# yoshihikosuzuki/ClassPro

Hardware: AMD Instinct MI355X
Metric: Mbases/s classified (k=40, 40x HiFi) at 1/2/4/8 MI355X vs CPU -T16 (higher is better)
Workload: dtype u16/f64

## Files before the change

classpro_amd/csrc/capi.hip:

```cpp
#include <hip/hip_runtime.h>
#include <stdio.h>
#include <stdlib.h>
#include <string.h>
#include <string>
#include <mutex>
#include <vector>
#include <chrono>
#include <thread>
#include <type_traits>
#include <time.h>
#include "cp_host_setup.h"
#include "kernels.hip"

static thread_local std::string g_err;
static int set_err(int code, const std::string &msg) { g_err = msg; return code; }

#define HIPCHK(call)                                                                       \
  do { hipError_t e_ = (call);                                                             \
       if (e_ != hipSuccess)                                                               \
         return set_err(CP_EHIP,std::string(#call)+": "+hipGetErrorString(e_));            \
     } while (0)
static int launch_status() { HIPCHK(hipGetLastError()); return CP_OK; }

extern "C" const char *cp_last_error(void) { return g_err.c_str(); }
// ... 964 lines not shown
  unsigned long long z[4] = { 0, 0, 0, 0 };
  HIPCHK(hipMemcpyToSymbol(HIP_SYMBOL(g_bounds),z,sizeof(z)));
  return CP_OK;
}
#endif

#if defined(CP_SEED_DEBUG) || defined(CP_SEED_DEBUG_TAKES)
extern "C" int cp_debug_seed_set(int read)
{ HIPCHK(hipMemcpyToSymbol(HIP_SYMBOL(g_seed_dbg_read),&read,sizeof(int))); return CP_OK; }
extern "C" int cp_debug_seed_get(int *out4, int *recs)
{ HIPCHK(hipDeviceSynchronize());
  HIPCHK(hipMemcpyFromSymbol(out4,HIP_SYMBOL(g_seed_dbg_n),16));
  HIPCHK(hipMemcpyFromSymbol(recs,HIP_SYMBOL(g_seed_dbg),8192*16));
  return CP_OK;
}
#endif
#if defined(CP_SEED_PROF) || defined(CP_PROF_WALK)
static int prof_read(unsigned long long *out, const void *sym, size_t n, bool reset = true)
{ static const unsigned long long z[12] = {0};
  HIPCHK(hipMemcpyFromSymbol(out,sym,n*sizeof(unsigned long long)));
  if (reset) HIPCHK(hipMemcpyToSymbol(sym,z,n*sizeof(unsigned long long)));
  return CP_OK;
}
#endif
#ifdef CP_SEED_PROF
extern "C" int cp_debug_seed_prof(unsigned long long *out8)
{ HIPCHK(hipDeviceSynchronize()); return prof_read(out8,HIP_SYMBOL(g_seed_prof),8); }
#endif
extern "C" int cp_debug_task_counts(cp_workspace *ws, int32_t *out, int64_t nreads)
{ if (!ws || !out || nreads < 0 || nreads > ws->nreads || ws->b.fwc.cap < (size_t)nreads*16)
    return set_err(CP_EINVAL,"cp_debug_task_counts: bad arguments");
  HIPCHK(hipDeviceSynchronize());
  if (nreads > 0) HIPCHK(hipMemcpy(out,ws->b.fwc.p,(size_t)nreads*4*sizeof(int32_t),hipMemcpyDeviceToHost));
  return CP_OK;
}
extern "C" int cp_debug_flag_bytes(cp_workspace *ws, int64_t *out2)
{ if (!ws || !out2) return set_err(CP_EINVAL,"cp_debug_flag_bytes: bad arguments");
  HIPCHK(hipDeviceSynchronize());
  const dbuf *arr[2] = { &ws->b.wall, &ws->b.wall_s };
  for (int a = 0; a < 2; a++)
    { std::vector<uint8_t> h(arr[a]->cap);
      if (arr[a]->cap) HIPCHK(hipMemcpy(h.data(),arr[a]->p,arr[a]->cap,hipMemcpyDeviceToHost));
      int64_t n = 0;
      for (uint8_t v : h) n += v != 0;
      out2[a] = n;
    }
  return CP_OK;
}
#ifdef CP_PROF_WALK
extern "C" int cp_debug_live_prof(unsigned long long *out8)
{ HIPCHK(hipDeviceSynchronize()); return prof_read(out8,HIP_SYMBOL(g_live_prof),8); }
extern "C" int cp_debug_emit_prof(unsigned long long *out8)
{ HIPCHK(hipDeviceSynchronize()); return prof_read(out8,HIP_SYMBOL(g_emit_prof),8); }
extern "C" int cp_debug_unrel_prof(unsigned long long *out8)
{ HIPCHK(hipDeviceSynchronize()); return prof_read(out8,HIP_SYMBOL(g_unrel_prof),8); }
extern "C" int cp_debug_rel_prof(unsigned long long *out12)
{ HIPCHK(hipDeviceSynchronize()); return prof_read(out12,HIP_SYMBOL(g_rel_prof),12); }
extern "C" int cp_debug_phase_prof(unsigned long long *out36)
{ HIPCHK(hipDeviceSynchronize());
  CHK(prof_read(out36,HIP_SYMBOL(g_phase_max),12));
  CHK(prof_read(out36+12,HIP_SYMBOL(g_phase_sum),12));
  return prof_read(out36+24,HIP_SYMBOL(g_phase_arg),12,false);
}
#endif

#include "kmer_table.hip"

#include "kmer_counts.hip"

#include "kmer_sort.hip"

#include "kmer_lookup.hip"

#include "kmer_hits.hip"

#include "kmer_runs.hip"

#include "kmer_setops.hip"

#include "kmer_cmphist.hip"

#include "kmer_hetpairs.hip"

#include "label_tools.hip"
```

classpro_amd/csrc/kernels.hip:

```cpp
#include <hip/hip_runtime.h>
#include <stdint.h>
#include <type_traits>
#include "cp_wall.h"
#include "cp_class.h"
#include "cp_seed.h"

#ifdef CP_BOUNDS
__device__ unsigned long long g_bounds[4];
#endif
#define WAVE 64
#define REL_MAXM 1024
#define UNREL_MAXN 1024
#ifndef REL_SMALL_MAXM
#define REL_SMALL_MAXM 112
#endif
#ifndef UNREL_SMALL_MAXN
#define UNREL_SMALL_MAXN 256
#endif
#define GRP_MAX_PLEN 65535

__device__ __forceinline__ void wave_sync() { __syncthreads(); }
__device__ __forceinline__ void wave_sync_lds()
{ __builtin_amdgcn_fence(__ATOMIC_RELEASE,"wavefront"); __builtin_amdgcn_wave_barrier(); __builtin_amdgcn_fence(__ATOMIC_ACQUIRE,"wavefront"); }

// ... 630 lines not shown
            }
          if (mv != ~0ull) break;
        }
      if (nx > 0 && !done && !flush_x(right ? 0x7fffffff : -1)) return;
      if (!done && (right ? plen < jend : jend == 0))
        { const double pe = pe_i * pe_i;
          if (pe >= CP_PE_THRES_FINAL)
            { if (*midx >= R->ecap) { R->overflow = 1; return; }
              ev.wave_grow(*midx);
              if (lane == 0)
                { cp_eintvl x; x.b = right ? i : 0; x.e = right ? plen : i; x.pe = pe;
                  ev.put(*midx,x);
                  F.fo[q] |= CP_W_PAIRED_M;
                }
              (*midx)++;
              if (*midx >= plen) { R->overflow = 8; return; }
            }
        }
      wave_sync();
    }
}

#define CP_PCLS(e,a)   (((uint32_t)(e) << 3) | ((uint32_t)(a) & 7u))
#define CP_PCLS_END(x) ((int)((x) >> 3))
#define CP_PCLS_CLS(x) (((x) & 7u) == 7u ? -1 : (int)((x) & 7u))

struct cp_rrec { int32_t b, e; uint16_t ccb, cce; int32_t idx; double pe; };
static_assert(sizeof(cp_rrec) == 24,"compact reliable-interval record");
struct cp_ivA { int32_t b, e; uint16_t cb, ce, ccb, cce; };
struct cp_ivB { double pe, peo_b, peo_e; };
struct cp_ivC { uint8_t is_rel; int8_t asgn; };
static_assert(sizeof(cp_ivA) == 16 && sizeof(cp_ivB) == 24 && sizeof(cp_ivC) == 2,"interval records as arrays");
struct cp_soa { cp_ivA *a; cp_ivB *b; cp_ivC *c; };
__device__ __forceinline__ void cp_soa_put(const cp_soa &S, int64_t at, const cp_intvl &I)
{ cp_ivA a; a.b = I.b; a.e = I.e; a.cb = I.cb; a.ce = I.ce; a.ccb = I.ccb; a.cce = I.cce;
  cp_ivB b; b.pe = I.pe; b.peo_b = I.peo_b; b.peo_e = I.peo_e;
  cp_ivC c; c.is_rel = I.is_rel; c.asgn = I.asgn;
  S.a[at] = a; S.b[at] = b; S.c[at] = c;
}
__device__ __forceinline__ cp_intvl cp_soa_get(const cp_soa &S, int64_t at)
{ const cp_ivA a = S.a[at]; const cp_ivB b = S.b[at]; const cp_ivC c = S.c[at];
  cp_intvl I;
  memset(&I,0,sizeof(I));
  I.b = a.b; I.e = a.e; I.cb = a.cb; I.ce = a.ce; I.ccb = a.ccb; I.cce = a.cce;
  I.is_rel = c.is_rel; I.asgn = c.asgn; I.pe = b.pe; I.peo_b = b.peo_b; I.peo_e = b.peo_e;
  return I;
}

#ifdef CP_PROF_WALK
__device__ unsigned long long g_phase_max[12], g_phase_sum[12], g_phase_arg[12];
__device__ unsigned long long g_live_prof[8];
__device__ unsigned long long g_unrel_prof[8];
__device__ unsigned long long g_emit_prof[8];
#ifdef CP_PROF_INNER
#define EM_LT0() unsigned long long em_t = wall_clock64()
#define EM_LT(k) do { unsigned long long t_ = wall_clock64(); if (lane == 0) atomicAdd(&g_emit_prof[k],t_-em_t); em_t = wall_clock64(); } while (0)
#endif
#define PH_STAMP(k) do { if (lane == 0) { unsigned long long t_ = wall_clock64(); unsigned long long d_ = t_-ph_t; ph_t = t_; \
      atomicAdd(&g_phase_sum[k],d_); unsigned long long o_ = atomicMax(&g_phase_max[k],d_); if (d_ > o_) g_phase_arg[k] = ((unsigned long long)r << 32) | (unsigned)n_c; } } while (0)
#elif defined(CP_STOP_AT)
#define PH_STAMP(k) do { if ((k) == CP_STOP_AT) { PH_STOP_EXTRA; return; } } while (0)
#else
#define PH_STAMP(k) ((void)0)
#endif
#ifndef EM_LT0
#define EM_LT0() ((void)0)
#define EM_LT(k) ((void)0)
#endif
#define PH_STOP_EXTRA

struct task_res { double own_pe, lc_v, hc_pe; int lc_j, hc;  };

#define FW_SEQ_WIN    32
#define FW_SEQ_STRIDE 36
struct cp_seq_lwin
  { CP_SEQ_T g; CP_LDS_PTR(const char) w; int lo, len;
    __device__ __forceinline__ char operator[](int p) const
    { const unsigned d = (unsigned)(p-lo); return d < (unsigned)len ? w[d] : g[p]; }
  };
__device__ __forceinline__ int cp_seq_dirword(const cp_seq_lwin &sq, int rlen, int pos, int dir, uint64_t *D)
{ (void)rlen;
  const int d = (dir > 0 ? pos : pos-7)-sq.lo;
  if (d < 0 || d+8 > sq.len) return 0;
  CP_LDS_PTR(const uint32_t) rw = (CP_LDS_PTR(const uint32_t))(sq.w+(d & ~3));
  const uint32_t x0 = rw[0], x1 = rw[1], x2 = rw[2];
  const uint32_t sh = (uint32_t)(d & 3)*8;
  const uint32_t lo = __builtin_amdgcn_alignbit(x1,x0,sh), hi = __builtin_amdgcn_alignbit(x2,x1,sh);
  const uint64_t x = (uint64_t)lo | ((uint64_t)hi << 32);
  *D = dir > 0 ? x : __builtin_bswap64(x);
  return 8;
}
struct __attribute__((packed, aligned(1))) cp_u8x16 { uint32_t v[4]; };
struct __attribute__((packed, aligned(1))) cp_u8x4 { uint32_t v; };
struct cp_seq_rwin
  { CP_SEQ_T g;
    uint64_t wl, wh;
    int lo, len;
    __device__ __forceinline__ char operator[](int p) const
    { const unsigned d = (unsigned)(p-lo);
      if (d < (unsigned)len)
        { const uint64_t x = (d < 8) ? wl : wh;
          return (char)(x >> ((d & 7)*8));
        }
      return g[p];
    }
  };
__device__ __forceinline__ int cp_seq_dirword(const cp_seq_rwin &sq, int rlen, int pos, int dir, uint64_t *D)
{ (void)rlen;
  const int d = (dir > 0 ? pos : pos-7)-sq.lo;
  if (sq.len != 16 || d < 0 || d > 8) return 0;
  const uint64_t x = d == 0 ? sq.wl : d == 8 ? sq.wh : (sq.wl >> (8*d)) | (sq.wh << (64-8*d));
  *D = dir > 0 ? x : __builtin_bswap64(x);
  return 8;
}
struct cp_seq_rsrc { CP_SEQ_T g; };
__device__ __forceinline__ cp_seq_rwin cp_seq_window(const cp_seq_rsrc &src, int pos, int rlen, int dir)
{ cp_seq_rwin sq;
  int lo = dir > 0 ? pos-7 : pos-11;
  if (lo > rlen-16) lo = rlen-16;
  if (lo < 0) lo = 0;
  sq.g = src.g; sq.lo = lo; sq.len = 0; sq.wl = sq.wh = 0;
  if (rlen-lo >= 16)
    { const cp_u8x16 x = *reinterpret_cast<const cp_u8x16 *>(CP_SPAN(src.g,lo,16));
      sq.wl = (uint64_t)x.v[0] | ((uint64_t)x.v[1] << 32);
// ... 51 lines not shown
  R.seq.g = CP_SEQ_VIEW(seq+seq_off[r],rlen); R.seq.w = (CP_LDS_PTR(const char))(s_win+lane*FW_SEQ_STRIDE); R.seq.lo = 0; R.seq.len = 0;
  R.wall = wall_all+po+r; R.wall_s = R.wall;
  R.eintvl = R.ointvl = nullptr; R.ecap = 0; R.eidx = R.oidx = 0; R.overflow = 0;
  cp_read_t<cp_perr_hybrid,cp_seq_rwin> R1;
  R1.P = P; R1.prof = R.prof; R1.lf = P->logfact; R1.plen = plen; R1.rlen = rlen;
  R1.wall = R.wall; R1.wall_s = R.wall; R1.eintvl = R1.ointvl = nullptr; R1.ecap = 0; R1.eidx = R1.oidx = 0; R1.overflow = 0;
  const int icap = (int)(ioff[r+1]-ioff[r]);
  int32_t *wl = wlist+ioff[r]*4;
  task_res *tres = tres_all+ioff[r];
  uint8_t *wall = R.wall;
  int32_t *cinfo = wl, *clist = wl+icap, *ccnt = wl+2*(int64_t)icap, *tlist = wl+3*(int64_t)icap;
  int n_c = 0;
#ifdef CP_PROF_WALK
  unsigned long long ph_t = wall_clock64();
#endif
  if (plen > 1)
    { const int64_t lo = po+1, hi = po+plen;
      const int64_t w_lo = lo >> 6, w_hi = (hi-1) >> 6;
      for (int64_t wb = w_lo; wb <= w_hi; wb += WAVE)
        { const int64_t w = wb+lane;
          const uint64_t bits = (w <= w_hi) ? bitmap_word(bm,w,lo,hi) : 0ull;
          int c = __popcll(bits), off = c;
          for (int o = 1; o < WAVE; o <<= 1)
            { int x = __shfl_up(off,o); if (lane >= o) off += x; }
          const int tot = __shfl(off,WAVE-1);
          off = n_c+off-c;
          for (uint64_t t = bits; t; t &= t-1)
            { const int k = __ffsll((long long)t)-1;
              if (off < icap) clist[off] = (int)((w << 6)+k-po);
              if (off < FW_LISTS) s_cl[off] = (int)((w << 6)+k-po);
              off++;
            }
          n_c += tot;
        }
    }
  if (n_c > icap) n_c = icap;
  const bool lists = n_c <= FW_LISTS;
  if (lists) wave_sync_lds(); else wave_sync();
  PH_STAMP(0);
  int n_t = 0, n_live0 = 0;
  for (int base = 0; base < n_c; base += WAVE)
    { int f0 = 0, f1 = 0;
      if (!lists) { if (base+lane < n_c) s_cl[lane] = clist[base+lane]; wave_sync_lds(); }
      if (base+lane < n_c)
        { const int i = s_cl[lists ? base+lane : lane];
          const bool drop = R.prof[i-1] > R.prof[i];
          cp_seq_rsrc rs; rs.g = R.seq.g;
          R1.seq = cp_seq_window(rs,drop ? i+P->K-2 : i,rlen,drop ? -1 : +1);
          cp_wall_pre pre;
          cp_wall_candidate_pre(&R1,i,&pre);
          f0 = cp_wall_candidate_filter(P,CP_SELF,pre);
          f1 = cp_wall_candidate_filter(P,CP_OTHERS,pre);
          cinfo[base+lane] = pre.maxt*32+pre.maxl+(f0 << 8)+(f1 << 12);
          ccnt[base+lane] = (int)R.prof[i-1] | ((int)R.prof[i] << 16);
          if (lists)
            { s_ci[base+lane] = (uint16_t)(pre.maxt*32+pre.maxl+(f0 << 8)+(f1 << 12));
              s_cc[base+lane] = (int)R.prof[i-1] | ((int)R.prof[i] << 16);
            }
        }
      const int l0 = (f0 & CP_CF_LIVE) ? 1 : 0, l1 = (f1 & CP_CF_LIVE) ? 1 : 0;
      int c = l0+l1, off = c;
      for (int o = 1; o < WAVE; o <<= 1)
        { int x = __shfl_up(off,o); if (lane >= o) off += x; }
      const int tot = __shfl(off,WAVE-1);
      off = n_t+off-c;
      if (l0) { if (off < icap) tlist[off] = (base+lane)*2;   if (lists) s_tl[off] = (uint16_t)((base+lane)*2);   off++; }
      if (l1) { if (off < icap) tlist[off] = (base+lane)*2+1; if (lists) s_tl[off] = (uint16_t)((base+lane)*2+1); }
      n_t += tot;
      n_live0 += __popcll(__ballot(l0));
    }
  int ovf = 0;
  if (n_t > icap) { ovf = 1; n_t = 0; n_c = 0; }
  if (lists) wave_sync_lds(); else wave_sync();
  PH_STAMP(7);
  for (int tb = 0; tb < n_t; tb += WAVE)
    { const int nb = (n_t-tb < WAVE) ? n_t-tb : WAVE;
      if (lane < nb)
        { if (!lists)
            { const int code = tlist[tb+lane], k = code >> 1;
              s_tl[lane] = (uint16_t)(lane*2+(code & 1)); s_cl[lane] = clist[k]; s_ci[lane] = (uint16_t)cinfo[k]; s_cc[lane] = ccnt[k];
            }
          const int code = s_tl[lists ? tb+lane : lane], k = code >> 1, e = code & 1;
          const int i = s_cl[k], tl = s_ci[k] & 255, cc = s_cc[k];
          cp_wall_pre pre;
          const int cim1 = cc & 0xffff, ci = (cc >> 16) & 0xffff;
          pre.cng = cim1 > ci ? cim1-ci : ci-cim1;
          if (cim1 > ci) { pre.wtype = CP_DROP; pre.cin = ci;   pre.cout = cim1; }
          else           { pre.wtype = CP_GAIN; pre.cin = cim1; pre.cout = ci;   }
          pre.maxt = tl >> 5; pre.maxl = tl & 31;
          pre.maxpe = P->pe[pre.maxt][pre.maxl];
          pre.lpe   = P->lpe[pre.maxt][pre.maxl];
          pre.l1mpe = P->l1mpe[pre.maxt][pre.maxl];
          cp_cand_pure c;
          cp_wall_candidate_live(&R,i,e,pre,&c,[&]() { fr_seq_win_load(R.seq,s_win+lane*FW_SEQ_STRIDE,cim1 > ci ? i+P->K-16 : i-24,rlen); });
          task_res q;
          q.own_pe = c.own_pe; q.lc_v = c.lc_v; q.hc_pe = c.hc_pe;
          q.lc_j = c.lc_j;
          q.hc = c.lc_kind | (c.hc_j >= 0 ? 4 : 0) | ((c.hc_j >= 0 ? c.hc_j-i : 0) << 16);
          tres[tb+lane] = q;
        }
    }
  PH_STAMP(6);
  if (lane == 0) { fwc[4*(int64_t)r] = n_c; fwc[4*(int64_t)r+1] = n_t; fwc[4*(int64_t)r+2] = n_live0; fwc[4*(int64_t)r+3] = ovf; }
}

#undef PH_STOP_EXTRA
#define PH_STOP_EXTRA
#ifndef FW2_WAVES_PER_EU
#define FW2_WAVES_PER_EU 5
#endif
__global__ void __launch_bounds__(WAVE) __attribute__((amdgpu_waves_per_eu(FW2_WAVES_PER_EU)))
k_find_wall(const cp_dev_params *__restrict__ P, const char *__restrict__ seq, const int64_t *__restrict__ seq_off,
            const uint16_t *__restrict__ prof, const int64_t *__restrict__ prof_off, int nreads,
            uint8_t *__restrict__ wall_all, uint8_t *__restrict__ walls_all,
            int32_t *__restrict__ hkeys, double *__restrict__ hvals, const int64_t *__restrict__ hoff,
            cp_eintvl *__restrict__ eintvl_all, cp_eintvl *__restrict__ ointvl_all, const int64_t *__restrict__ eoff,
            cp_intvl *__restrict__ intvl_all, const int64_t *__restrict__ ioff,
            int32_t *__restrict__ nintvl, int32_t *__restrict__ err, const int32_t *__restrict__ perm,
            int32_t *__restrict__ wlist, const task_res *__restrict__ tres_all, const int32_t *__restrict__ fwc,
            cp_intvl *__restrict__ rintvl_all, int32_t *__restrict__ relmap_all, int32_t *__restrict__ nrel, int do_rel,
            cp_rrec *__restrict__ rrec_all, cp_soa soa)
{ if ((int)blockIdx.x >= nreads) return;
  const int r = perm[blockIdx.x];
  const int lane = lane_id();
  const int64_t po = prof_off[r];
  const int plen = (int)(prof_off[r+1]-po);
  const int rlen = (int)(seq_off[r+1]-seq_off[r]);

#ifndef FW_XCAP
#define FW_XCAP 8
#endif
#ifndef FW_LCAP1
#define FW_LCAP1 64
#endif
  if (plen <= 0)
    { if (lane == 0) { nintvl[r] = 0; if (do_rel) nrel[r] = 0; }
      return;
    }
  constexpr int LCAP0 = 256, LCAP1 = FW_LCAP1;
  __shared__ int32_t s_mkey[LCAP0+LCAP1];
  __shared__ double  s_mval[LCAP0+LCAP1];
  __shared__ uint16_t s_x[FW_XCAP];
  __shared__ int s_nx;
  __shared__ cp_eintvl s_ev[FW_EVL];
  cp_read_t<cp_perr_hybrid,CP_SEQ_T,CP_PROF_T,const double *,fw_evl> R;
  R.P = P; R.prof = CP_PROF_VIEW(prof+po,plen); R.seq = CP_SEQ_VIEW(seq+seq_off[r],rlen); R.lf = P->logfact; R.plen = plen; R.rlen = rlen;
  R.wall = wall_all+po+r;
  R.wall_s = walls_all+po+r;
  { const int64_t ho = hoff[r], hc = (hoff[r+1]-ho) >> 1;
    R.perror.g.keys = hkeys+ho;
    R.perror.g.vals = hvals+ho*4;
    R.perror.g.mask = (uint32_t)hc-1;
    R.perror.lkeys = (CP_LDS_PTR(int32_t))s_mkey;
    R.perror.lvals = (CP_LDS_PTR(double))s_mval;
    R.perror.lcap0 = LCAP0; R.perror.lcap1 = LCAP1;
    R.perror.use_lds = 0;
  }
  if (lane == 0) s_nx = 0;
  for (int k = lane; k < LCAP0+LCAP1; k += WAVE)
    s_mkey[k] = -1;
  R.eintvl.g = eintvl_all+eoff[r];
  R.eintvl.l = (CP_LDS_PTR(cp_eintvl))s_ev;
  R.ointvl.g = ointvl_all+eoff[r];
  R.ecap = (int)(eoff[r+1]-eoff[r]);
  R.eidx = R.oidx = 0; R.overflow = 0;
  cp_intvl *intvl = intvl_all+ioff[r];
  const int icap = (int)(ioff[r+1]-ioff[r]);
  int32_t *wl = wlist+ioff[r]*4;
  const task_res *tres = tres_all+ioff[r];
  uint8_t *wall = R.wall;
  const uint8_t *wall_s = R.wall_s;
  __shared__ task_res s_res[WAVE];
  int32_t *clist = wl+icap, *ccnt = wl+2*(int64_t)icap, *tlist = wl+3*(int64_t)icap;
  const int n_c = fwc[4*(int64_t)r], n_t = fwc[4*(int64_t)r+1], n_live0 = fwc[4*(int64_t)r+2];
  if (fwc[4*(int64_t)r+3]) R.overflow = 1;
#ifdef CP_PROF_WALK
  unsigned long long ph_t = wall_clock64();
#endif
  R.perror.use_lds = ((2*n_live0 <= LCAP0-8) ? 1 : 0) | ((2*(n_t-n_live0) <= LCAP1-8) ? 2 : 0);
  R.eintvl.big = (n_live0 > FW_EVL || R.ecap < FW_EVL) ? 1 : 0;
  { const int hc = (int)R.perror.g.mask+1;
    for (int e = 0; e < 2; e++)
      if (!((R.perror.use_lds >> e) & 1))
        for (int k = lane; k < hc; k += WAVE) R.perror.g.keys[(size_t)e*hc+k] = -1;
  }
  wave_sync();
  int *sbuf = reinterpret_cast<int *>(s_res);
  constexpr int SBUF = (int)(sizeof(task_res)*WAVE/sizeof(int));
  constexpr int SCOMP = 64;
  constexpr int U16 = 2*(SBUF-2*SCOMP);
  uint16_t *s16 = reinterpret_cast<uint16_t *>(sbuf);
  fw_cflags F;
  F.pos = s16; F.fo = reinterpret_cast<uint8_t *>(s16+n_c); F.fs = F.fo+n_c; F.n = n_c;
  constexpr int NDEP = 128;
  static_assert(sizeof(task_res)*WAVE >= 4*256+NDEP*sizeof(unsigned long long),"flags of 255 candidates and the dependency masks fit the staging block");
  bool onchip = R.perror.use_lds == 3 && plen <= 65535 && n_c <= 255 && 3*n_c+2*SCOMP+1 <= U16 && !R.eintvl.big;
  const int32_t *cinfo = wl;
  auto flags_to_hbm = [&]()
    { for (int q = lane; q < n_c; q += WAVE)
        if ((cinfo[q] >> 12) & CP_CF_WALLNOW) wall[clist[q]] = CP_W_WALL_O;
      wave_sync();
    };
  if (R.perror.use_lds == 3)
    { unsigned long long *s_dep = reinterpret_cast<unsigned long long *>(s_res)+(sizeof(task_res)*WAVE/sizeof(unsigned long long)-NDEP);
      const uint64_t ltm = (1ull << lane)-1;
      const int ecap = R.ecap;
      const bool ebig = R.eintvl.big != 0;
      int eidx = 0, oidx = 0, ovf = 0;
      auto memo_cell = [&](int pos, int e, int w) -> int
        { const int key = pos*2+w, off = e ? LCAP0 : 0;
          const uint32_t m = (uint32_t)(e ? LCAP1 : LCAP0)-1;
          uint32_t h = ((uint32_t)key*0x9E3779B1u >> 9) & m;
          while (true)
            { const int32_t k = s_mkey[off+h];
              if (k == key) break;
              if (k < 0)
                { const int32_t o = atomicCAS(&s_mkey[off+h],-1,key);
                  if (o == -1) { s_mval[off+h] = -INFINITY; break; }
                  if (o == key) break;
                }
              h = (h+1) & m;
            }
          return off+(int)h;
        };
      for (;;)
        { if (onchip)
            { for (int q = lane; q < n_c; q += WAVE)
                { F.pos[q] = (uint16_t)clist[q]; F.fo[q] = ((cinfo[q] >> 12) & CP_CF_WALLNOW) ? CP_W_WALL_O : 0; F.fs[q] = 0; }
              wave_sync();
            }
          else flags_to_hbm();
          bool bail = false;
          for (int tb = 0; tb < n_t; tb += WAVE)
            { const int nb = (n_t-tb < WAVE) ? n_t-tb : WAVE;
              bool open = lane < nb;
              int pos = 1, kc = 0, e = 0, w = 0, lc_j = -1, lc_kind = CP_LC_NONE, hc_j = -1;
              double own_pe = 0., lc_v = 0., hc_pe = 0.;
              if (open)
                { const int code = tlist[tb+lane], k = code >> 1, cc = ccnt[k];
                  const task_res q = tres[tb+lane];
                  pos = clist[k]; kc = k; e = code & 1;
                  w = (cc & 0xffff) > ((cc >> 16) & 0xffff) ? CP_DROP : CP_GAIN;
                  own_pe = q.own_pe; lc_v = q.lc_v; hc_pe = q.hc_pe;
                  lc_j = q.lc_j; lc_kind = q.hc & 3;
                  hc_j = (q.hc & 4) ? pos+(q.hc >> 16) : -1;
                }
              const int p1 = (lc_kind == CP_LC_PAIR || lc_kind == CP_LC_BOUNDARY) ? lc_j : -1, p2 = hc_j;
              for (int q = lane; q < NDEP; q += WAVE) s_dep[q] = 0ull;
              wave_sync();
              const int s0 = (int)((uint32_t)(pos*2+e)*0x9E3779B1u >> 25), s1 = (int)((uint32_t)(p1*2+e)*0x9E3779B1u >> 25),
                        s2 = (int)((uint32_t)(p2*2+e)*0x9E3779B1u >> 25);
              if (open)
                { atomicOr(&s_dep[s0],1ull << lane);
                  if (p1 >= 0) atomicOr(&s_dep[s1],1ull << lane);
                  if (p2 >= 0) atomicOr(&s_dep[s2],1ull << lane);
                }
              wave_sync();
              uint64_t dep = 0;
              if (open)
                { dep = s_dep[s0];
                  if (p1 >= 0) dep |= s_dep[s1];
                  if (p2 >= 0) dep |= s_dep[s2];
                  dep &= ltm;
                }
              { const int k0 = open ? pos*2+e : -2, k1 = (open && p1 >= 0) ? p1*2+e : -1, k2 = (open && p2 >= 0) ? p2*2+e : -1;
                uint64_t rem = dep, keep = 0;
                while (__ballot(rem != 0))
                  { const int u = rem ? __ffsll((long long)rem)-1 : lane;
                    const int a0 = __shfl(k0,u), a1 = __shfl(k1,u), a2 = __shfl(k2,u);
                    const bool hit = a0 == k0 || a0 == k1 || a0 == k2
                                     || (a1 >= 0 && (a1 == k0 || a1 == k1 || a1 == k2))
                                     || (a2 >= 0 && (a2 == k0 || a2 == k1 || a2 == k2));
                    if (rem) { if (hit) keep |= 1ull << u; rem &= rem-1; }
                  }
                dep = keep;
              }
              bool hasE = false, hasO = false, off_list = false;
              cp_eintvl I; I.b = I.e = 0; I.pe = 0.;
#ifdef CP_PROF_WALK
              {
                uint64_t depx = 0;
                const int k0 = pos*2+e, k1 = p1 >= 0 ? p1*2+e : -1, k2 = p2 >= 0 ? p2*2+e : -1;
                for (int u = 0; u < WAVE; u++)
                  { const int a0 = __shfl(k0,u), a1 = __shfl(k1,u), a2 = __shfl(k2,u);
                    const bool uo = __shfl((int)open,u) != 0;
                    if (uo && u < lane && (a0 == k0 || (k1 >= 0 && a0 == k1) || (k2 >= 0 && a0 == k2)
                                          || (a1 >= 0 && (a1 == k0 || a1 == k1 || a1 == k2)) || (a2 >= 0 && (a2 == k0 || a2 == k1 || a2 == k2))))
                      depx |= 1ull << u;
                  }
                int rh = 0, rx = 0;
                bool oh = open, ox = open;
                for (uint64_t um = __ballot(oh); um; um = __ballot(oh)) { if (oh && (dep & um) == 0) oh = false; rh++; }
                for (uint64_t um = __ballot(ox); um; um = __ballot(ox)) { if (ox && (depx & um) == 0) ox = false; rx++; }
                if (lane == 0) { atomicAdd(&g_live_prof[0],(unsigned long long)rh); atomicAdd(&g_live_prof[1],(unsigned long long)rx); atomicAdd(&g_live_prof[2],1ull); atomicAdd(&g_live_prof[3],(unsigned long long)nb); }
              }
#endif
              for (uint64_t um = __ballot(open); um; um = __ballot(open))
                { if (open && (dep & um) == 0)
                    { open = false;
                      const uint8_t fl = onchip ? ((e == CP_SELF) ? F.fs[kc] : F.fo[kc]) : ((e == CP_SELF) ? R.wall_s[pos] : wall[pos]);
                      if (!(fl & (e == CP_SELF ? CP_W_PAIRED_S : CP_W_PAIRED_O)))
                        { const int ci = memo_cell(pos,e,w);
// ... 50 lines not shown
                                      hasO = true;
                                    }
                                }
                            }
                          if (!accept && e == CP_OTHERS)
                            { if (onchip) F.fo[kc] = fl | CP_W_WALL_O; else wall[pos] = fl | CP_W_WALL_O; }
                        }
                    }
                  wave_sync();
                }
              if (__ballot(off_list)) bail = true;
              const uint64_t mE = __ballot(hasE), mO = __ballot(hasO);
              if (hasE)
                { const int sl = eidx+__popcll(mE & ltm);
                  if (sl < ecap) { if (ebig) R.eintvl.g[sl] = I; else R.eintvl.l[sl] = I; }
                }
              if (hasO)
                { const int sl = oidx+__popcll(mO & ltm);
                  if (sl < ecap) R.ointvl.g[sl] = I;
                }
              eidx += __popcll(mE); oidx += __popcll(mO);
              if (eidx > ecap) { eidx = ecap; ovf = 1; }
              if (oidx > ecap) { oidx = ecap; ovf = 1; }
            }
          wave_sync();
          if (bail)
            {
#ifdef CP_PROF_WALK
              if (lane == 0) atomicAdd(&g_live_prof[6],1ull);
#endif
              for (int q = lane; q < n_c; q += WAVE)
                { const int i = F.pos[q];
                  if (F.fo[q]) wall[i] = F.fo[q];
                  if (F.fs[q]) R.wall_s[i] = F.fs[q];
                }
              if (lane < FW_XCAP) R.wall_s[s_x[lane]] = (CP_W_WALL_S|CP_W_PAIRED_S);
              onchip = false;
              wave_sync();
            }
          break;
        }
      if (lane < 2) { R.eidx = lane == 0 ? eidx : 0; R.oidx = lane == 1 ? oidx : 0; R.overflow |= ovf; }
    }
  else
  {
  flags_to_hbm();
  if (lane < 2)
    { R.use_win = (P->K+24+CP_MAX_N_HC < 128) ? 1 : 0;
      R.win_base = 0; R.win_lo = R.win_hi = 0;
      R.spec_wallnow = 1;
    }
  for (int tb = 0; tb < n_t; tb += WAVE)
    { const int nb = (n_t-tb < WAVE) ? n_t-tb : WAVE;
      int code_l = 0, cc_l = 0, pos_l = 1;
      if (lane < nb)
        { const int code = tlist[tb+lane], k = code >> 1;
          code_l = code; cc_l = ccnt[k]; pos_l = clist[k];
          s_res[lane] = tres[tb+lane];
        }
      wave_sync();
      for (int k = 0; k < nb; k++)
        { const int code = __builtin_amdgcn_readlane(code_l,k), cc = __builtin_amdgcn_readlane(cc_l,k);
          const int pos = __builtin_amdgcn_readlane(pos_l,k);
          if (lane == (code & 1))
            { cp_cand_pure c;
              const task_res &q = s_res[k];
              c.flags = CP_CF_LIVE;
              c.own_pe = q.own_pe; c.lc_v = q.lc_v; c.hc_pe = q.hc_pe;
              c.lc_j = q.lc_j; c.lc_kind = q.hc & 3;
              c.hc_j = (q.hc & 4) ? pos+(q.hc >> 16) : -1;
              cp_wall_candidate_replay(&R,pos,lane,(cc & 0xffff) > ((cc >> 16) & 0xffff) ? CP_DROP : CP_GAIN,c);
            }
        }
      wave_sync();
    }
  }
  R.use_win = 0; R.spec_wallnow = 0;
  int n_x = 0;
  if (onchip)
    { n_x = __builtin_amdgcn_readfirstlane(s_nx);
      if (n_x > FW_XCAP) n_x = FW_XCAP;
      if (lane == 0)
        for (int a = 1; a < n_x; a++)
          { const uint16_t v = s_x[a];
            int b = a-1;
            while (b >= 0 && s_x[b] > v) { s_x[b+1] = s_x[b]; b--; }
            s_x[b+1] = v;
          }
      wave_sync();
    }
  PH_STAMP(1);
  int NS = __shfl(R.eidx,0), NO = __shfl(R.oidx,1);
  int overflow = __shfl(R.overflow,0) | __shfl(R.overflow,1);
  R.eidx = NS; R.oidx = NO;
  wave_sync();

  int *s_cb = sbuf+SBUF-2*SCOMP, *s_ce = sbuf+SBUF-SCOMP;
  const bool on16 = plen <= 65535 && 2*n_c+2*SCOMP+1 <= U16;
  R.eintvl.big = __shfl(R.eintvl.big,0);
  if (onchip)
    { for (int k = lane; k < NO; k += WAVE)
        { const cp_eintvl o = R.ointvl.g[k];
          const int kb = cf_find(F,o.b), ke = cf_find(F,o.e);
          if (kb >= 0) F.fo[kb] &= (uint8_t)~(CP_W_WALL_O|CP_W_PAIRED_O);
          if (ke >= 0) F.fo[ke] &= (uint8_t)~(CP_W_WALL_O|CP_W_PAIRED_O);
        }
    }
  else if (lane == 0)
    for (int k = 0; k < NO; k++)
      { const cp_eintvl o = R.ointvl.g[k];
        wall[o.b] &= ~(CP_W_WALL_O|CP_W_PAIRED_O);
        wall[o.e] &= ~(CP_W_WALL_O|CP_W_PAIRED_O);
      }
  wave_sync();
  bool cf = onchip;
  if (!cf && plen <= 65535 && n_c <= 255 && 3*n_c+2*SCOMP+1 <= U16 && !R.eintvl.big)
    { for (int q = lane; q < n_c; q += WAVE)
        { const int i = clist[q];
          F.pos[q] = (uint16_t)i; F.fo[q] = wall[i]; F.fs[q] = wall_s[i];
        }
      wave_sync();
      bool miss = false;
      for (int k = lane; k < NS; k += WAVE)
        miss = miss || cf_find(F,R.eintvl.b(k)) < 0 || cf_find(F,R.eintvl.e(k)) < 0;
// ... 322 lines not shown
                    xe = __builtin_amdgcn_ds_permute(tA*4,e0);
                    xc = __builtin_amdgcn_ds_permute(tA*4,c0);
                    xk = base+__builtin_amdgcn_ds_permute(tA*4,lane);
                    act = lane < n0;
                  }
                if (useB)
                  { const int yb = __builtin_amdgcn_ds_permute(tB*4,b1);
                    const int ye = __builtin_amdgcn_ds_permute(tB*4,e1);
                    const int yc = __builtin_amdgcn_ds_permute(tB*4,c1);
                    const int yk = base+WAVE+__builtin_amdgcn_ds_permute(tB*4,lane);
                    if (lane >= offB && lane < offB+n1) { xb = yb; xe = ye; xc = yc; xk = yk; act = true; }
                  }
                int res = 0;
                if (act)
                  { cp_seq_rsrc rs; rs.g = R.seq;
                    int ccb, cce;
                    const bool rel = cp_rel_counts(P,R.prof,rs,rs,rlen,xb,xe,xc & 0xffff,(xc >> 16) & 0xffff,xk,&ccb,&cce);
                    res = ccb | (cce << 16) | (rel ? 0x8000 : 0);
                  }
                if (useA) { const int g = __builtin_amdgcn_ds_bpermute(tA*4,res); if (p0) res0 = g; }
                if (useB) { const int g = __builtin_amdgcn_ds_bpermute(tB*4,res); if (p1) res1 = g; }
              }
          }
        EM_LT(2);
        auto put = [&](int k, int b, int e, int c, double pe, int res) __attribute__((always_inline))
          { const bool ok = (res & 0x8000) != 0;
            const uint16_t ccb = (uint16_t)(res & 0x7fff), cce = (uint16_t)((res >> 16) & 0x7fff);
            if (k < Ncl)
              { if (aos && res) { intvl[k].ccb = ccb; intvl[k].cce = cce; intvl[k].is_rel = ok ? 1 : 0; }
                if (use_soa)
                  { cp_ivA qa; qa.b = b; qa.e = e; qa.cb = (uint16_t)(c & 0xffff); qa.ce = (uint16_t)((c >> 16) & 0xffff); qa.ccb = ccb; qa.cce = cce;
                    cp_ivC qc; qc.is_rel = ok ? 1 : 0; qc.asgn = CP_N_STATE;
                    soa.a[ioff[r]+k] = qa; soa.c[ioff[r]+k] = qc;
                  }
              }
            if (do_rel)
              { const uint64_t mask = __ballot(ok);
                if (ok)
                  { const int rank = __popcll(mask & ((1ull << lane)-1));
                    if (do_rel == 2)
                      { cp_rrec q; q.b = b; q.e = e; q.ccb = ccb; q.cce = cce; q.idx = k; q.pe = pe;
                        rrec_all[ioff[r]+M+rank] = q;
                      }
                    else
                      { rintvl[M+rank] = intvl[k];
                        relmap[M+rank] = k;
                      }
                  }
                M += __popcll(mask);
              }
          };
        put(k0,b0,e0,c0,pe0,res0);
        if (base+WAVE < Ncl) put(k1,b1,e1,c1,pe1,res1);
        EM_LT(4);
      }
    if (do_rel && lane == 0) nrel[r] = M;
    if (do_rel == 2 && (M > REL_SMALL_MAXM || plen > GRP_MAX_PLEN))
      { wave_sync();
        const cp_rrec *rr = rrec_all+ioff[r];
        for (int i = lane; i < M; i += WAVE)
          { const int k = rr[i].idx;
            rintvl[i] = aos ? intvl[k] : cp_soa_get(soa,ioff[r]+k);
            relmap[i] = k;
          }
      }
  }
  PH_STAMP(5);
  wave_sync();
#ifdef CP_PROF_WALK
  if (lane == 0) { atomicAdd(&g_live_prof[4],R.perror.use_lds == 3 ? 1ull : 0ull); atomicAdd(&g_live_prof[5],onchip ? 1ull : 0ull); atomicAdd(&g_live_prof[7],cf ? 1ull : 0ull); }
#endif
  if (onchip) { }
  else if (overflow)
    { for (int j = lane; j <= plen; j += WAVE) { wall[j] = 0; R.wall_s[j] = 0; } }
  else
    { for (int q = lane; q < n_c; q += WAVE)
        { const int i = clist[q]; wall[i] = 0; R.wall_s[i] = 0; }
      for (int k = lane; k < NS; k += WAVE)
        { const int b = R.eintvl.b(k), e = R.eintvl.e(k);
          wall[b] = 0; wall[e] = 0; R.wall_s[b] = 0; R.wall_s[e] = 0;
        }
    }
  if (lane == 0)
    { nintvl[r] = (N > icap) ? icap : N;
      if (overflow) atomicOr(err,overflow);
    }
}

__global__ void __launch_bounds__(WAVE)
k_find_rel(const cp_dev_params *__restrict__ P, const char *__restrict__ seq, const int64_t *__restrict__ seq_off,
           const uint16_t *__restrict__ prof, const int64_t *__restrict__ prof_off, int nreads,
           cp_intvl *__restrict__ intvl_all, cp_intvl *__restrict__ rintvl_all, int32_t *__restrict__ relmap_all,
           const int64_t *__restrict__ ioff, const int32_t *__restrict__ nintvl, int32_t *__restrict__ nrel)
{ const int r = blockIdx.x;
  if (r >= nreads) return;
  const int lane = lane_id();
  const int N = nintvl[r];
  const int rlen = (int)(seq_off[r+1]-seq_off[r]);
  const CP_PROF_T pr = CP_PROF_VIEW(prof+prof_off[r],rlen-(P->K-1));
  const CP_SEQ_T sq = CP_SEQ_VIEW(seq+seq_off[r],rlen);
  cp_intvl *intvl = intvl_all+ioff[r], *rintvl = rintvl_all+ioff[r];
  int32_t *relmap = relmap_all+ioff[r];
  __shared__ __attribute__((aligned(4))) char s_ctx[WAVE*FR_STRIDE];
  int M = 0;
  for (int base = 0; base < N; base += WAVE)
    { int idx = base+lane;
      bool ok = false;
// ... 1716 lines not shown
```

Before: 373,400.

## Pack task metadata into task_res and prefetch first-wave walk inputs early

Widens task_res with pos, kc, e and wall-type bits so the walk kernel no longer makes the dependent tlist→ccnt→clist global loads per task. It also skips the tlist/ccnt global writes when the LDS lists are used. Per-read offsets and fwc counts are loaded once and pinned to scalar registers. The first chunk of tres, clist and cinfo is prefetched before the LDS/HBM initialisation so those loads overlap with the clears. The staging LDS block is decoupled from the task_res size, and the profiling macros are reworked, with a risk of breaking EM_LT when profiling is on.

```diff
diff --git a/classpro_amd/csrc/capi.hip b/classpro_amd/csrc/capi.hip
--- a/classpro_amd/csrc/capi.hip
+++ b/classpro_amd/csrc/capi.hip
@@ -1040,6 +1040,8 @@
 { HIPCHK(hipDeviceSynchronize()); return prof_read(out8,HIP_SYMBOL(g_live_prof),8); }
 extern "C" int cp_debug_emit_prof(unsigned long long *out8)
 { HIPCHK(hipDeviceSynchronize()); return prof_read(out8,HIP_SYMBOL(g_emit_prof),8); }
+extern "C" int cp_debug_fw_prof(unsigned long long *out12)
+{ HIPCHK(hipDeviceSynchronize()); return prof_read(out12,HIP_SYMBOL(g_fw_prof),12); }
 extern "C" int cp_debug_unrel_prof(unsigned long long *out8)
 { HIPCHK(hipDeviceSynchronize()); return prof_read(out8,HIP_SYMBOL(g_unrel_prof),8); }
 extern "C" int cp_debug_rel_prof(unsigned long long *out12)
diff --git a/classpro_amd/csrc/kernels.hip b/classpro_amd/csrc/kernels.hip
--- a/classpro_amd/csrc/kernels.hip
+++ b/classpro_amd/csrc/kernels.hip
@@ -706,10 +706,9 @@
 __device__ unsigned long long g_live_prof[8];
 __device__ unsigned long long g_unrel_prof[8];
 __device__ unsigned long long g_emit_prof[8];
-#ifdef CP_PROF_INNER
+__device__ unsigned long long g_fw_prof[12];
 #define EM_LT0() unsigned long long em_t = wall_clock64()
-#define EM_LT(k) do { unsigned long long t_ = wall_clock64(); if (lane == 0) atomicAdd(&g_emit_prof[k],t_-em_t); em_t = wall_clock64(); } while (0)
-#endif
+#define EM_LT(k) do { unsigned long long t_ = wall_clock64(); if (lane == 0) atomicAdd(&g_fw_prof[4+(k)],t_-em_t); em_t = wall_clock64(); } while (0)
 #define PH_STAMP(k) do { if (lane == 0) { unsigned long long t_ = wall_clock64(); unsigned long long d_ = t_-ph_t; ph_t = t_; \
       atomicAdd(&g_phase_sum[k],d_); unsigned long long o_ = atomicMax(&g_phase_max[k],d_); if (d_ > o_) g_phase_arg[k] = ((unsigned long long)r << 32) | (unsigned)n_c; } } while (0)
 #elif defined(CP_STOP_AT)
@@ -723,7 +722,13 @@
 #endif
 #define PH_STOP_EXTRA
 
-struct task_res { double own_pe, lc_v, hc_pe; int lc_j, hc;  };
+struct task_res { double own_pe, lc_v, hc_pe; int lc_j, hc, pos, kc; };
+#define TR_E(hc)     (((hc) >> 3) & 1)
+#define TR_WTYPE(hc) (((hc) >> 4) & 1)
+static_assert(sizeof(task_res) == 40,"three doubles and four ints, no padding");
+static_assert(CP_DROP == 0 && CP_GAIN == 1 && CP_SELF == 0 && CP_OTHERS == 1,"one bit each in task_res::hc");
+static_assert(CP_LC_REJECT <= 3,"lc_kind takes two bits of task_res::hc");
+struct task_stage { double own_pe, lc_v, hc_pe; int lc_j, hc; };
 
 #define FW_SEQ_WIN    32
 #define FW_SEQ_STRIDE 36
@@ -881,7 +886,7 @@
           f0 = cp_wall_candidate_filter(P,CP_SELF,pre);
           f1 = cp_wall_candidate_filter(P,CP_OTHERS,pre);
           cinfo[base+lane] = pre.maxt*32+pre.maxl+(f0 << 8)+(f1 << 12);
-          ccnt[base+lane] = (int)R.prof[i-1] | ((int)R.prof[i] << 16);
+          if (!lists) ccnt[base+lane] = (int)R.prof[i-1] | ((int)R.prof[i] << 16);
           if (lists)
             { s_ci[base+lane] = (uint16_t)(pre.maxt*32+pre.maxl+(f0 << 8)+(f1 << 12));
               s_cc[base+lane] = (int)R.prof[i-1] | ((int)R.prof[i] << 16);
@@ -893,8 +898,8 @@
         { int x = __shfl_up(off,o); if (lane >= o) off += x; }
       const int tot = __shfl(off,WAVE-1);
       off = n_t+off-c;
-      if (l0) { if (off < icap) tlist[off] = (base+lane)*2;   if (lists) s_tl[off] = (uint16_t)((base+lane)*2);   off++; }
-      if (l1) { if (off < icap) tlist[off] = (base+lane)*2+1; if (lists) s_tl[off] = (uint16_t)((base+lane)*2+1); }
+      if (l0) { if (lists) s_tl[off] = (uint16_t)((base+lane)*2);   else if (off < icap) tlist[off] = (base+lane)*2;   off++; }
+      if (l1) { if (lists) s_tl[off] = (uint16_t)((base+lane)*2+1); else if (off < icap) tlist[off] = (base+lane)*2+1; }
       n_t += tot;
       n_live0 += __popcll(__ballot(l0));
     }
@@ -925,7 +930,11 @@
           task_res q;
           q.own_pe = c.own_pe; q.lc_v = c.lc_v; q.hc_pe = c.hc_pe;
           q.lc_j = c.lc_j;
-          q.hc = c.lc_kind | (c.hc_j >= 0 ? 4 : 0) | ((c.hc_j >= 0 ? c.hc_j-i : 0) << 16);
+          int code2;
+          if (lists) code2 = s_tl[tb+lane]; else code2 = tlist[tb+lane];
+          q.hc = c.lc_kind | (c.hc_j >= 0 ? 4 : 0) | ((code2 & 1) << 3) | ((int)pre.wtype << 4)
+                 | ((c.hc_j >= 0 ? c.hc_j-i : 0) << 16);
+          q.pos = i; q.kc = code2 >> 1;
           tres[tb+lane] = q;
         }
     }
@@ -952,15 +961,22 @@
 { if ((int)blockIdx.x >= nreads) return;
   const int r = perm[blockIdx.x];
   const int lane = lane_id();
-  const int64_t po = prof_off[r];
-  const int plen = (int)(prof_off[r+1]-po);
-  const int rlen = (int)(seq_off[r+1]-seq_off[r]);
+  const int64_t po = prof_off[r], po1 = prof_off[r+1], so = seq_off[r], so1 = seq_off[r+1];
+  const int64_t ho = hoff[r], ho1 = hoff[r+1], eo = eoff[r], eo1 = eoff[r+1], io = ioff[r], io1 = ioff[r+1];
+  const int4 fw4 = *reinterpret_cast<const int4 *>(fwc+4*(int64_t)r);
+  asm volatile("" :: "s"(po), "s"(po1), "s"(so), "s"(so1), "s"(ho), "s"(ho1), "s"(eo), "s"(eo1), "s"(io), "s"(io1),
+                     "s"(fw4.x), "s"(fw4.y), "s"(fw4.z), "s"(fw4.w));
+  const int plen = (int)(po1-po);
+  const int rlen = (int)(so1-so);
 
 #ifndef FW_XCAP
 #define FW_XCAP 8
 #endif
 #ifndef FW_LCAP1
 #define FW_LCAP1 64
+#endif
+#ifdef CP_PROF_WALK
+  const unsigned long long fw_t0 = wall_clock64();
 #endif
   if (plen <= 0)
     { if (lane == 0) { nintvl[r] = 0; if (do_rel) nrel[r] = 0; }
@@ -973,10 +989,10 @@
   __shared__ int s_nx;
   __shared__ cp_eintvl s_ev[FW_EVL];
   cp_read_t<cp_perr_hybrid,CP_SEQ_T,CP_PROF_T,const double *,fw_evl> R;
-  R.P = P; R.prof = CP_PROF_VIEW(prof+po,plen); R.seq = CP_SEQ_VIEW(seq+seq_off[r],rlen); R.lf = P->logfact; R.plen = plen; R.rlen = rlen;
+  R.P = P; R.prof = CP_PROF_VIEW(prof+po,plen); R.seq = CP_SEQ_VIEW(seq+so,rlen); R.lf = P->logfact; R.plen = plen; R.rlen = rlen;
   R.wall = wall_all+po+r;
   R.wall_s = walls_all+po+r;
-  { const int64_t ho = hoff[r], hc = (hoff[r+1]-ho) >> 1;
+  { const int64_t hc = (ho1-ho) >> 1;
     R.perror.g.keys = hkeys+ho;
     R.perror.g.vals = hvals+ho*4;
     R.perror.g.mask = (uint32_t)hc-1;
@@ -985,54 +1001,77 @@
     R.perror.lcap0 = LCAP0; R.perror.lcap1 = LCAP1;
     R.perror.use_lds = 0;
   }
-  if (lane == 0) s_nx = 0;
-  for (int k = lane; k < LCAP0+LCAP1; k += WAVE)
-    s_mkey[k] = -1;
-  R.eintvl.g = eintvl_all+eoff[r];
+  R.eintvl.g = eintvl_all+eo;
   R.eintvl.l = (CP_LDS_PTR(cp_eintvl))s_ev;
-  R.ointvl.g = ointvl_all+eoff[r];
-  R.ecap = (int)(eoff[r+1]-eoff[r]);
+  R.ointvl.g = ointvl_all+eo;
+  R.ecap = (int)(eo1-eo);
   R.eidx = R.oidx = 0; R.overflow = 0;
-  cp_intvl *intvl = intvl_all+ioff[r];
-  const int icap = (int)(ioff[r+1]-ioff[r]);
-  int32_t *wl = wlist+ioff[r]*4;
-  const task_res *tres = tres_all+ioff[r];
+  cp_intvl *intvl = intvl_all+io;
+  const int icap = (int)(io1-io);
+  int32_t *wl = wlist+io*4;
+  const task_res *tres = tres_all+io;
   uint8_t *wall = R.wall;
   const uint8_t *wall_s = R.wall_s;
-  __shared__ task_res s_res[WAVE];
-  int32_t *clist = wl+icap, *ccnt = wl+2*(int64_t)icap, *tlist = wl+3*(int64_t)icap;
-  const int n_c = fwc[4*(int64_t)r], n_t = fwc[4*(int64_t)r+1], n_live0 = fwc[4*(int64_t)r+2];
-  if (fwc[4*(int64_t)r+3]) R.overflow = 1;
+  constexpr int SBLK = 2048;
+  __shared__ unsigned long long s_blk[SBLK/8];
+  int32_t *clist = wl+icap;
+  const int n_c = fw4.x, n_t = fw4.y, n_live0 = fw4.z;
+  if (fw4.w) R.overflow = 1;
 #ifdef CP_PROF_WALK
   unsigned long long ph_t = wall_clock64();
 #endif
   R.perror.use_lds = ((2*n_live0 <= LCAP0-8) ? 1 : 0) | ((2*(n_t-n_live0) <= LCAP1-8) ? 2 : 0);
   R.eintvl.big = (n_live0 > FW_EVL || R.ecap < FW_EVL) ? 1 : 0;
-  { const int hc = (int)R.perror.g.mask+1;
-    for (int e = 0; e < 2; e++)
-      if (!((R.perror.use_lds >> e) & 1))
-        for (int k = lane; k < hc; k += WAVE) R.perror.g.keys[(size_t)e*hc+k] = -1;
-  }
-  wave_sync();
-  int *sbuf = reinterpret_cast<int *>(s_res);
-  constexpr int SBUF = (int)(sizeof(task_res)*WAVE/sizeof(int));
+  int *sbuf = reinterpret_cast<int *>(s_blk);
+  constexpr int SBUF = SBLK/(int)sizeof(int);
   constexpr int SCOMP = 64;
   constexpr int U16 = 2*(SBUF-2*SCOMP);
   uint16_t *s16 = reinterpret_cast<uint16_t *>(sbuf);
   fw_cflags F;
   F.pos = s16; F.fo = reinterpret_cast<uint8_t *>(s16+n_c); F.fs = F.fo+n_c; F.n = n_c;
   constexpr int NDEP = 128;
-  static_assert(sizeof(task_res)*WAVE >= 4*256+NDEP*sizeof(unsigned long long),"flags of 255 candidates and the dependency masks fit the staging block");
+  static_assert(SBLK >= 4*256+NDEP*sizeof(unsigned long long),"flags of 255 candidates and the dependency masks fit the staging block");
+  static_assert(sizeof(task_stage)*WAVE <= SBLK,"a chunk of the one-lane replay fits the staging block");
   bool onchip = R.perror.use_lds == 3 && plen <= 65535 && n_c <= 255 && 3*n_c+2*SCOMP+1 <= U16 && !R.eintvl.big;
   const int32_t *cinfo = wl;
+  unsigned long long *s_dep = s_blk+(SBLK/8-NDEP);
+  int cl_r[4] = { 0, 0, 0, 0 }, ci_r[4] = { 0, 0, 0, 0 };
+  task_res qr = { 0., 0., 0., -1, 0, 1, 0 };
+  if (R.perror.use_lds == 3)
+    { if (onchip)
+        {
+#pragma unroll
+          for (int j = 0; j < 4; j++)
+            if (j*WAVE+lane < n_c) { cl_r[j] = clist[j*WAVE+lane]; ci_r[j] = cinfo[j*WAVE+lane]; }
+        }
+      if (lane < n_t) qr = tres[lane];
+    }
+  if (lane == 0) s_nx = 0;
+  for (int k = lane; k < LCAP0+LCAP1; k += WAVE)
+    s_mkey[k] = -1;
+  if (R.perror.use_lds == 3)
+    for (int q = lane; q < NDEP; q += WAVE) s_dep[q] = 0ull;
+  { const int hc = (int)R.perror.g.mask+1;
+    for (int e = 0; e < 2; e++)
+      if (!((R.perror.use_lds >> e) & 1))
+        for (int k = lane; k < hc; k += WAVE) R.perror.g.keys[(size_t)e*hc+k] = -1;
+  }
+  if (R.perror.use_lds == 3 && onchip)
+    {
+#pragma unroll
+      for (int j = 0; j < 4; j++)
+        { const int q = j*WAVE+lane;
+          if (q < n_c) { F.pos[q] = (uint16_t)cl_r[j]; F.fo[q] = ((ci_r[j] >> 12) & CP_CF_WALLNOW) ? CP_W_WALL_O : 0; F.fs[q] = 0; }
+        }
+    }
+  wave_sync();
   auto flags_to_hbm = [&]()
     { for (int q = lane; q < n_c; q += WAVE)
         if ((cinfo[q] >> 12) & CP_CF_WALLNOW) wall[clist[q]] = CP_W_WALL_O;
       wave_sync();
     };
   if (R.perror.use_lds == 3)
-    { unsigned long long *s_dep = reinterpret_cast<unsigned long long *>(s_res)+(sizeof(task_res)*WAVE/sizeof(unsigned long long)-NDEP);
-      const uint64_t ltm = (1ull << lane)-1;
+    { const uint64_t ltm = (1ull << lane)-1;
       const int ecap = R.ecap;
       const bool ebig = R.eintvl.big != 0;
       int eidx = 0, oidx = 0, ovf = 0;
@@ -1053,30 +1092,36 @@
           return off+(int)h;
         };
       for (;;)
-        { if (onchip)
-            { for (int q = lane; q < n_c; q += WAVE)
-                { F.pos[q] = (uint16_t)clist[q]; F.fo[q] = ((cinfo[q] >> 12) & CP_CF_WALLNOW) ? CP_W_WALL_O : 0; F.fs[q] = 0; }
-              wave_sync();
-            }
-          else flags_to_hbm();
+        { if (!onchip) flags_to_hbm();
           bool bail = false;
+#ifdef CP_PROF_WALK
+          if (lane == 0) { atomicAdd(&g_fw_prof[0],wall_clock64()-fw_t0); atomicAdd(&g_fw_prof[3],1ull); }
+#endif
           for (int tb = 0; tb < n_t; tb += WAVE)
             { const int nb = (n_t-tb < WAVE) ? n_t-tb : WAVE;
               bool open = lane < nb;
+#ifdef CP_PROF_WALK
+              const unsigned long long fw_t1 = wall_clock64();
+#endif
               int pos = 1, kc = 0, e = 0, w = 0, lc_j = -1, lc_kind = CP_LC_NONE, hc_j = -1;
               double own_pe = 0., lc_v = 0., hc_pe = 0.;
               if (open)
-                { const int code = tlist[tb+lane], k = code >> 1, cc = ccnt[k];
-                  const task_res q = tres[tb+lane];
-                  pos = clist[k]; kc = k; e = code & 1;
-                  w = (cc & 0xffff) > ((cc >> 16) & 0xffff) ? CP_DROP : CP_GAIN;
+                { if (tb > 0) qr = tres[tb+lane];
+                  const task_res &q = qr;
+                  pos = q.pos; kc = q.kc; e = TR_E(q.hc); w = TR_WTYPE(q.hc);
                   own_pe = q.own_pe; lc_v = q.lc_v; hc_pe = q.hc_pe;
                   lc_j = q.lc_j; lc_kind = q.hc & 3;
                   hc_j = (q.hc & 4) ? pos+(q.hc >> 16) : -1;
                 }
+#ifdef CP_PROF_WALK
+              asm volatile("" :: "v"(pos), "v"(kc), "v"(e), "v"(w), "v"(lc_j), "v"(lc_kind), "v"(hc_j), "v"(own_pe), "v"(lc_v), "v"(hc_pe));
+              if (lane == 0) { atomicAdd(&g_fw_prof[1],wall_clock64()-fw_t1); atomicAdd(&g_fw_prof[2],1ull); }
+#endif
               const int p1 = (lc_kind == CP_LC_PAIR || lc_kind == CP_LC_BOUNDARY) ? lc_j : -1, p2 = hc_j;
-              for (int q = lane; q < NDEP; q += WAVE) s_dep[q] = 0ull;
-              wave_sync();
+              if (tb > 0)
+                { for (int q = lane; q < NDEP; q += WAVE) s_dep[q] = 0ull;
+                  wave_sync();
+                }
               const int s0 = (int)((uint32_t)(pos*2+e)*0x9E3779B1u >> 25), s1 = (int)((uint32_t)(p1*2+e)*0x9E3779B1u >> 25),
                         s2 = (int)((uint32_t)(p2*2+e)*0x9E3779B1u >> 25);
               if (open)
@@ -1233,24 +1278,26 @@
     }
   for (int tb = 0; tb < n_t; tb += WAVE)
     { const int nb = (n_t-tb < WAVE) ? n_t-tb : WAVE;
-      int code_l = 0, cc_l = 0, pos_l = 1;
+      task_stage *s_st = reinterpret_cast<task_stage *>(s_blk);
+      int hc_l = 0, pos_l = 1;
       if (lane < nb)
-        { const int code = tlist[tb+lane], k = code >> 1;
-          code_l = code; cc_l = ccnt[k]; pos_l = clist[k];
-          s_res[lane] = tres[tb+lane];
+        { const task_res q = tres[tb+lane];
+          hc_l = q.hc; pos_l = q.pos;
+          task_stage t; t.own_pe = q.own_pe; t.lc_v = q.lc_v; t.hc_pe = q.hc_pe; t.lc_j = q.lc_j; t.hc = q.hc;
+          s_st[lane] = t;
         }
       wave_sync();
       for (int k = 0; k < nb; k++)
-        { const int code = __builtin_amdgcn_readlane(code_l,k), cc = __builtin_amdgcn_readlane(cc_l,k);
+        { const int hc = __builtin_amdgcn_readlane(hc_l,k);
           const int pos = __builtin_amdgcn_readlane(pos_l,k);
-          if (lane == (code & 1))
+          if (lane == TR_E(hc))
             { cp_cand_pure c;
-              const task_res &q = s_res[k];
+              const task_stage &q = s_st[k];
               c.flags = CP_CF_LIVE;
               c.own_pe = q.own_pe; c.lc_v = q.lc_v; c.hc_pe = q.hc_pe;
-              c.lc_j = q.lc_j; c.lc_kind = q.hc & 3;
-              c.hc_j = (q.hc & 4) ? pos+(q.hc >> 16) : -1;
-              cp_wall_candidate_replay(&R,pos,lane,(cc & 0xffff) > ((cc >> 16) & 0xffff) ? CP_DROP : CP_GAIN,c);
+              c.lc_j = q.lc_j; c.lc_kind = hc & 3;
+              c.hc_j = (hc & 4) ? pos+(hc >> 16) : -1;
+              cp_wall_candidate_replay(&R,pos,lane,TR_WTYPE(hc),c);
             }
         }
       wave_sync();
@@ -1679,7 +1726,7 @@
           };
         put(k0,b0,e0,c0,pe0,res0);
         if (base+WAVE < Ncl) put(k1,b1,e1,c1,pe1,res1);
-        EM_LT(4);
+        EM_LT(3);
       }
     if (do_rel && lane == 0) nrel[r] = M;
     if (do_rel == 2 && (M > REL_SMALL_MAXM || plen > GRP_MAX_PLEN))
```

New measurement: 379,500 (median of 6 runs). +1.7%, better.
